# iracigt/ceres-raytracer

Measured on AMD Instinct MI355X. Metric: Mrays/sec (primary+shadow) on dragon.obj 1920x1080; 1/2/4/8-GPU scaling, higher is better.
Workload: dtype f32; 1 GPU; dragon_1080: dragon.obj 1920x1080 primary+shadow, 16 copies of the config view per step; views=config, W=1920, H=1080, row_block=1080, parallelism=one GPU, whole frames, float_framebuffer=True, streams=8

## Files before the change

### ceres-raytracer_amd/csrc/ceres_types.hpp

```cpp
#pragma once
#include <cstddef>
#include <cstdint>
#include <vector>

namespace ceres {

struct Tri48 {
    float p0[3], e1[3], e2[3], n[3];
};
static_assert(sizeof(Tri48) == 48, "Tri48");

struct RefNode {
    float bounds[6];
    uint32_t primitive_count;
    uint32_t first_child_or_primitive;
};
static_assert(sizeof(RefNode) == 32, "RefNode");

struct alignas(16) SiblingPair {
    float lb[6];
    float rb[6];
    uint32_t lcount, lfirst;
    uint32_t rcount, rfirst;
};
// ... 67 lines not shown
    uint32_t error;
    unsigned long long hits;
    unsigned long long pairs;
    unsigned long long tests;
    uint32_t pad[24];
};
static_assert(sizeof(Shard) == 128, "Shard");

constexpr int kMaxFrames = 64;
constexpr int kFramesPerLaunch = 56;
struct FrameCam {
    float eye[3], dir[3], iu[3], iv[3], sun[3];
};

constexpr uint32_t kTileXBits = 13, kTileYBits = 13;
constexpr uint32_t pack_tile(uint32_t f, uint32_t y, uint32_t x) { return (f << (kTileXBits + kTileYBits)) | (y << kTileXBits) | x; }

struct CullRect { uint16_t i0, i1, j0, j1; };

struct KParams {
    FrameCam cam[kFramesPerLaunch];
    CullRect cull_rect[kFramesPerLaunch];
    uint32_t frames;
    uint32_t W, H;
    uint32_t row_block, rank, world, local_rows;
    uint32_t bands;
    uint32_t band_magic;
    uint32_t row_blocks_per_frame;
    uint32_t stack_entries;
    uint32_t root_leaf_count, root_leaf_first;
    float root_box[6];
    uint32_t root_box_ok;
    uint32_t cull;
    uint32_t shadow_stack_entries;
    uint32_t steal_first;
    uint32_t packets;
    uint32_t tiles_x;
    uint32_t lds_entries;
    uint32_t tile_packed;
    const uint32_t* tile_order;
    const SiblingPair* pairs;
    const Node4* nodes4;
    const QNode4* qnodes4;
    const Tri48* tris;
    const uint32_t* orig;
    const float* norms;
    float* pixels;
    uint8_t* rgb8;
    Shard* shards;
    int32_t* rec_prim;
    float* rec_tuv;
    int8_t* rec_shadow;
    unsigned long long* wave_log;
};
static_assert(sizeof(KParams) <= 4096, "KParams must fit the 4 KB kernel-argument limit");

struct DeviceLayout {
    float root_box[6] = {0, 0, 0, 0, 0, 0};
    SiblingPair* pairs = nullptr;
    Node4* nodes4 = nullptr;
    Tri48* tris = nullptr;
    uint32_t* orig = nullptr;
    size_t n_pairs = 0, n_nodes4 = 0;
    uint32_t depth = 0, stack4 = 0, root_leaf_count = 0, root_leaf_first = 0;
};
#ifdef __HIPCC__
int relayout_device(const Tri48* d_tris, uint32_t n_tri, const RefNode* d_nodes, uint32_t n_nodes, const uint32_t* d_prim,
                    hipStream_t stream, DeviceLayout& out);
#endif

int relayout_bvh(const RefNode* nodes, size_t n_nodes, const uint64_t* prim, size_t n_tri, const Tri48* tris,
                 std::vector<SiblingPair>& pairs, std::vector<Tri48>& leaf_tris, std::vector<uint32_t>& orig,
                 uint32_t& depth, uint32_t& root_leaf_count, uint32_t& root_leaf_first);
int build_shadow_bvh4(const std::vector<SiblingPair>& pairs, std::vector<Node4>& out, uint32_t& stack_bound,
                      uint32_t& not_collapsed);
int order_shadow_bvh4(std::vector<Node4>& nodes, uint32_t& first_bound);
int relayout_bvh64(const RefNode64* nodes, size_t n_nodes, const uint64_t* prim, size_t n_tri, const Tri96* tris,
                   std::vector<SiblingPair64>& pairs, std::vector<Tri96>& leaf_tris, std::vector<uint32_t>& orig,
                   uint32_t& depth, uint32_t& root_leaf_count, uint32_t& root_leaf_first);

}
```

### ceres-raytracer_amd/csrc/render_hip.hip

```cpp
#include <hip/hip_runtime.h>

#include <algorithm>
#include <chrono>
#include <cfloat>
#include <cmath>
#include <cstdint>
#include <cstdlib>
#include <cstring>
#include <new>
#include <string>
#include <type_traits>
#include <vector>

#include "ceres_render.h"
#include "ceres_types.hpp"
#include "host_common.hpp"
#include "pow24.hpp"

#pragma clang fp contract(off)

#ifndef CERES_COUNTING
#define CERES_COUNTING 0
#endif
#ifndef CERES_TILES_PER_WAVE
// ... 693 lines not shown
            --sp;
            m = (uint64_t(uint32_t(__builtin_amdgcn_readlane(s_hi, int(sp)))) << 32 |
                 uint32_t(__builtin_amdgcn_readlane(s_lo, int(sp)))) & ~occ;
            if (m) { cur = uint32_t(__builtin_amdgcn_readlane(s_node, int(sp))); break; }
        }
        if (!m) return occ;
    }
}

__device__ __forceinline__ uint8_t quantize(float x) {
    const float a = x * 255;
    const float m = (255.0f < a) ? 255.0f : a;
    const float q = (m < 0.0f) ? 0.0f : m;
    return static_cast<uint8_t>(static_cast<int>(q));
}

__device__ __forceinline__ void store_pixel(const KParams& P, uint32_t f, uint32_t lr, uint32_t i, float c0, float c1,
                                            float c2) {
    const size_t frame_base = size_t(f) * P.local_rows;
    CERES_COUNT_V(kFStoreV, (P.pixels ? 12u : 0u) + (P.rgb8 ? 3u : 0u));
    if (P.pixels) {
        float* q = P.pixels + 3 * ((frame_base + lr) * P.W + i);
        q[0] = c0; q[1] = c1; q[2] = c2;
    }
    if (P.rgb8) {
        uint8_t* q = P.rgb8 + 3 * ((frame_base + (P.local_rows - 1 - lr)) * P.W + i);
        q[0] = quantize(c0); q[1] = quantize(c1); q[2] = quantize(c2);
    }
}

template <bool kBands = false>
__device__ __forceinline__ uint32_t global_row(const KParams& P, uint32_t f, uint32_t lr) {
    if (P.world == 1) return lr;
    if constexpr (kBands) {
        const uint32_t x = P.rank + f, q = __umulhi(x, P.band_magic);
        return (x - q * P.world) * P.row_block + lr;
    }
    return ((lr / P.row_block) * P.world + P.rank) * P.row_block + lr % P.row_block;
}

template <bool kG = false>
__device__ __forceinline__ F3 primary_dir(const KParams& P, uint32_t f, uint32_t i, uint32_t j) {
    const float u = 2 * (float(i) + 0.5f) / float(P.W) - 1.0f;
    const float v = 2 * (float(j) + 0.5f) / float(P.H) - 1.0f;
    const FrameCam& c = P.cam[f];
    F3 a;
    if constexpr (kG)
        a = F3{c.dir[0] + __builtin_fmaf(c.iv[0], v, c.iu[0] * u), c.dir[1] + __builtin_fmaf(c.iv[1], v, c.iu[1] * u),
               c.dir[2] + __builtin_fmaf(c.iv[2], v, c.iu[2] * u)};
    else a = f3(c.iu) * u + f3(c.iv) * v + f3(c.dir);
    return kG ? normalizeG<kG>(a) : normalize(a);
}

__device__ __forceinline__ bool tile_misses_root(const KParams& P, uint32_t f, bool active, uint32_t i, uint32_t j) {
    const CullRect& r = P.cull_rect[f];
    const bool out = i < r.i0 || i > r.i1 || j < r.j0 || j > r.j1;
    return __ballot(active && !out) == 0;
}

template <bool kG>
__device__ __forceinline__ F3 hit_point(const TriV& tr, F3 normal, float hu, float hv) {
    const F3 p1 = tr.p0 - tr.e1, p2 = tr.p0 + tr.e2;
    const float scale = -0.00001;
    const float w = 1 - hu - hv;
    if constexpr (kG) {
        auto c = [&](float p0, float q1, float q2, float n) {
            return __builtin_fmaf(n, scale, __builtin_fmaf(w, q2, __builtin_fmaf(hv, q1, hu * p0)));
        };
        return {c(tr.p0.x, p1.x, p2.x, normal.x), c(tr.p0.y, p1.y, p2.y, normal.y), c(tr.p0.z, p1.z, p2.z, normal.z)};
    } else {
        F3 p = tr.p0 * hu + p1 * hv + p2 * w;
        return p + normal * scale;
    }
}

template <bool kG = false>
__device__ __forceinline__ void shade(F3 sun_line, const float* nrm, F3 view, float u, float v, float c[3]) {
    c[0] = c[1] = c[2] = 0.0f;
    const float amb = 0.2;
    const F3 vneg = view * -1.0f;
    const float w[3] = {u, v, 1 - u - v};
#pragma unroll
    for (int k = 0; k < 3; ++k) {
        const F3 N{nrm[3 * k], nrm[3 * k + 1], nrm[3 * k + 2]};
        const float lam = kG ? fabsf(dotA<true>(sun_line, N)) : fabsf(sun_line.x * N.x + sun_line.y * N.y + sun_line.z * N.z);
        const float spec = 0.8f * pow24f(dotA<kG>(N, normalizeG<kG>(sun_line + vneg)));
        const float base = kG ? __builtin_fmaf(lam, 0.5f, amb) : amb + 0.5f * lam;
        auto clamp01 = [](float x) { return (x < 0.f) ? 0.f : (1.f < x) ? 1.f : x; };
        auto ch = [&](float k) { return kG ? __builtin_fmaf(base, k, spec) : base * k + spec; };
        c[0] += w[k] * clamp01(ch(0.5f));
        c[1] += w[k] * clamp01(ch(0.0f));
        c[2] += w[k] * clamp01(ch(0.8f));
    }
}

__device__ __forceinline__ uint32_t wave_sum(uint32_t x) {
#pragma unroll
    for (int off = 32; off > 0; off >>= 1) x += __shfl_xor(x, off, 64);
    return x;
}

template <bool kStats, bool kRobust, bool kG>
__global__ __launch_bounds__(kBlock) void ceres_primary(const KParams P) {
    extern __shared__ __attribute__((aligned(16))) uint32_t lds[];
    const uint32_t tid = threadIdx.x, lane = tid & 63, wave = tid >> 6;
    uint32_t* stk = lds + tid;
    const uint32_t f = blockIdx.y / P.row_blocks_per_frame;
    const uint32_t by = blockIdx.y - f * P.row_blocks_per_frame;
    const uint32_t lx = lane & 7, ly = lane >> 3;
    const uint32_t i = blockIdx.x * 16 + (wave & 1) * 8 + lx;
    const uint32_t lr = by * 16 + (wave >> 1) * 8 + ly;
    const bool active = i < P.W && lr < P.local_rows;
    const uint32_t px = (f * P.local_rows + lr) * P.W + i;
    bool hit = false;
    Hit h{0, 0.f, 0.f, 0.f};
    uint32_t n_pairs = 0, n_tests = 0;
    bool overflow = false;
    const bool culled = !kStats && P.cull && tile_misses_root(P, f, active, i, global_row(P, f, lr));
    if (culled) {
        if (active) store_pixel(P, f, lr, i, 0.f, 0.f, 0.f);
    } else if (active) {
        const F3 view = primary_dir<kG>(P, f, i, global_row(P, f, lr));
        hit = guarded_trace<kStats, kBlock, uint32_t*, kRobust, -1, kG>(P, f3(P.cam[f].eye), view, stk, h, n_pairs, n_tests,
                                                                      overflow);
        if (P.rec_prim) {
            P.rec_prim[px] = hit ? int32_t(P.orig[h.slot]) : -1;
            P.rec_tuv[3 * size_t(px)] = hit ? h.t : 0.f;
            P.rec_tuv[3 * size_t(px) + 1] = hit ? h.u : 0.f;
            P.rec_tuv[3 * size_t(px) + 2] = hit ? h.v : 0.f;
            P.rec_shadow[px] = -1;
        }
        if (!hit) {
            store_pixel(P, f, lr, i, 0.f, 0.f, 0.f);
        } else {
            CERES_COUNT_V(kFShadeV, 48);
            const F3 normal = normalizeG<kG>(load_tri(P.tris + h.slot).n);
            store_pixel(P, f, lr, i, fabsf(normal.x), fabsf(normal.y), fabsf(normal.z));
        }
    }
    const uint32_t wave_id = (blockIdx.y * gridDim.x + blockIdx.x) * (kBlock / 64) + wave;
    const uint32_t shard = wave_id % kShards;
    const uint32_t nh = __popcll(__ballot(hit));
    if (lane == 0 && nh) atomicAdd(&P.shards[shard].hits, (unsigned long long)nh);
    if (kStats) {
        const uint32_t wp = wave_sum(n_pairs), wt = wave_sum(n_tests);
        if (lane == 0) {
            atomicAdd(&P.shards[shard].pairs, (unsigned long long)wp);
            atomicAdd(&P.shards[shard].tests, (unsigned long long)wt);
        }
    }
    if (overflow) atomicOr(&P.shards[shard].error, 1u);
}

#ifndef CERES_LEAN_WRITES
#define CERES_LEAN_WRITES 0
#endif
#ifndef CERES_FUSED_MINW16
#define CERES_FUSED_MINW16 7
#endif
#ifndef CERES_FUSED_MINW16_TPW4
#define CERES_FUSED_MINW16_TPW4 6
#endif
#ifndef CERES_FUSED_MINW16_SOLO
#define CERES_FUSED_MINW16_SOLO 7
#endif
#ifndef CERES_FUSED_MINW32
#define CERES_FUSED_MINW32 1
#endif
#ifndef CERES_STACK16
#define CERES_STACK16 1
#endif
#ifndef CERES_STACK24
#define CERES_STACK24 1
#endif
// ... 162 lines not shown
    return w;
}

template <typename StkT, bool kRobust, bool kQ, bool kG>
__device__ __forceinline__ bool shadow_packet(const KParams& P, bool hit, const RayWork& w, uint32_t lane, bool& blocked) {
    if constexpr (!kRobust && !kQ && CERES_SHADOW_PACKET && std::is_same<StkT, uint16_t*>::value) {
        const uint64_t act = __ballot(hit);
        if (!act) { blocked = false; return true; }
        const uint32_t oct = (__float_as_uint(w.ix) >> 31) | (__float_as_uint(w.iy) >> 31) << 1 |
                             (__float_as_uint(w.iz) >> 31) << 2;
        const int first = __builtin_ctzll(act);
        const uint32_t oct0 = uint32_t(__builtin_amdgcn_readlane(int(oct), first));
        const bool finite = isfinite(w.ix) && isfinite(w.iy) && isfinite(w.iz) && isfinite(w.sx) && isfinite(w.sy) &&
                            isfinite(w.sz);
        if (!P.packets || P.shadow_stack_entries > 64 || P.root_leaf_count || __ballot(hit && (oct != oct0 || !finite)))
            return false;
        auto bc = [&](float x) { return hit ? x : __int_as_float(__builtin_amdgcn_readlane(__float_as_int(x), first)); };
        const F3 o{bc(w.o.x), bc(w.o.y), bc(w.o.z)}, d{bc(w.d.x), bc(w.d.y), bc(w.d.z)};
        const Slab<false> sl{bc(w.ix), bc(w.iy), bc(w.iz), bc(w.sx), bc(w.sy), bc(w.sz), o};
        uint64_t occ = 0;
        switch (oct0) {
            case 0: occ = packet_any4<0, kG>(P, sl, o, d, act, lane); break;
            case 1: occ = packet_any4<1, kG>(P, sl, o, d, act, lane); break;
            case 2: occ = packet_any4<2, kG>(P, sl, o, d, act, lane); break;
            case 3: occ = packet_any4<3, kG>(P, sl, o, d, act, lane); break;
            case 4: occ = packet_any4<4, kG>(P, sl, o, d, act, lane); break;
            case 5: occ = packet_any4<5, kG>(P, sl, o, d, act, lane); break;
            case 6: occ = packet_any4<6, kG>(P, sl, o, d, act, lane); break;
            default: occ = packet_any4<7, kG>(P, sl, o, d, act, lane); break;
        }
        blocked = (occ >> lane) & 1u;
        return true;
    }
    return false;
}

template <bool kG, bool kBands = false>
__device__ __forceinline__ void shade_pixel(const KParams& P, uint32_t f, uint32_t lr, uint32_t i, uint32_t pix,
                                            bool blocked, F3 sun_line, uint32_t slot, float hu, float hv,
                                            uint32_t& occluded, float c[3]) {
    if (P.rec_shadow) P.rec_shadow[pix] = blocked ? 1 : 0;
    c[0] = c[1] = c[2] = 0.f;
    if (blocked) {
        ++occluded;
    } else {
        const F3 view = primary_dir<kG>(P, f, i, global_row<kBands>(P, f, lr));
        CERES_COUNT_V(kFShadeV, 40);
        shade<kG>(sun_line, P.norms + 9 * size_t(P.orig[slot]), view, hu, hv, c);
    }
}

constexpr int kFusedB = 64;
constexpr size_t kLdsPerCu = 160 * 1024;
__device__ __forceinline__ float fresh_zero() {
    float z;
    asm volatile("v_mov_b32 %0, 0" : "=v"(z));
    return z;
}

template <bool kStats, typename StkT, int kMinW, bool kRobust, bool kSteal, bool kQ, bool kG, int kTPWo = 0, bool kBands = false>
__global__ __launch_bounds__(kFusedB) __attribute__((amdgpu_waves_per_eu(kMinW))) void ceres_fused(const KParams P) {
    constexpr int kB = kFusedB;
    constexpr bool kPacketsCompiled = !kStats && !kSteal && !kRobust && !kQ && CERES_SHADOW_PACKET && std::is_same<StkT, uint16_t*>::value;
    extern __shared__ __attribute__((aligned(16))) uint32_t lds[];
    __shared__ StealLdsT<kB> L;
    const uint32_t lane = threadIdx.x, tid = lane;
    constexpr uint32_t kTPWp = (kStats || kSteal) ? 1 : kTPWo ? uint32_t(kTPWo) : uint32_t(CERES_TILES_PER_WAVE);
    constexpr bool kPair = CERES_PAIR_STORES && !kStats && !kSteal && kTPWp >= 2 && std::is_same<StkT, uint16_t*>::value;
    __shared__ typename std::conditional<kPair, PairStash, NoStash>::type S;
    auto tile_pixel = [&](uint32_t t, uint32_t& f_, uint32_t& lr_, uint32_t& i_) {
        uint32_t by_, bx_;
        if (P.tile_packed) {
            bx_ = t & ((1u << kTileXBits) - 1u);
            by_ = (t >> kTileXBits) & ((1u << kTileYBits) - 1u);
            f_ = t >> (kTileXBits + kTileYBits);
        } else {
            const uint32_t per_frame_ = P.tiles_x * P.row_blocks_per_frame;
            f_ = t / per_frame_;
            const uint32_t rem = t - f_ * per_frame_;
            by_ = rem / P.tiles_x; bx_ = rem - by_ * P.tiles_x;
        }
        const uint32_t lx = (lane & 1) | ((lane >> 1) & 2) | ((lane >> 2) & 4), ly = ((lane >> 1) & 1) | ((lane >> 2) & 2) | ((lane >> 3) & 4);
        i_ = bx_ * 8u + lx;
        lr_ = by_ * 8u + ly;
        return i_ < P.W && lr_ < P.local_rows && (!kBands || global_row<true>(P, f_, lr_) < P.H);
    };
    auto emit = [&](uint32_t q, bool last, uint32_t t_prev, bool act, uint32_t f_, uint32_t lr_, uint32_t i_, float c0, float c1,
                    float c2) {
        if constexpr (kPair) {
            if (!(q & 1u) && !last) {
                S.c[0][lane] = c0; S.c[1][lane] = c1; S.c[2][lane] = c2;
                return;
            }
            if (q & 1u) {
                uint32_t pf, plr, pi;
                if (tile_pixel(t_prev, pf, plr, pi)) store_pixel(P, pf, plr, pi, S.c[0][lane], S.c[1][lane], S.c[2][lane]);
            }
        }
        if (act) store_pixel(P, f_, lr_, i_, c0, c1, c2);
    };
    StkT stk;
    if constexpr (std::is_same<StkT, Stk24>::value)
        stk = Stk24{reinterpret_cast<uint16_t*>(lds) + tid,
                    reinterpret_cast<uint8_t*>(lds) + size_t(P.lds_entries) * kB * 2 + tid};
    else
        stk = reinterpret_cast<StkT>(lds) + tid;
    constexpr uint32_t kTile = 8;
    constexpr uint32_t kTPW = (kStats || kSteal) ? 1 : kTPWo ? uint32_t(kTPWo) : uint32_t(CERES_TILES_PER_WAVE);
    const uint32_t per_frame = P.tiles_x * P.row_blocks_per_frame;
    const uint32_t n_tiles = per_frame * P.frames;
    uint32_t n_shadow = 0, occluded = 0, n_pairs = 0, n_tests = 0;
    bool overflow = false;
    static_assert(kTPW == 1 || kTPW == 2 || kTPW == 4 || kTPW == 8, "CERES_TILES_PER_WAVE must be 1, 2, 4 or 8");
    uint4 tiles4 = make_uint4(0, 0, 0, 0), tiles4b = make_uint4(0, 0, 0, 0);
    if constexpr (kTPW == 8) {
        tiles4 = sload_u4(P.tile_order + 8 * size_t(blockIdx.x), 0);
        tiles4b = sload_u4(P.tile_order + 8 * size_t(blockIdx.x), 1);
    } else if constexpr (kTPW == 4) {
        tiles4 = sload_u4(P.tile_order + 4 * size_t(blockIdx.x), 0);
    } else if constexpr (kTPW == 2) {
        tiles4.x = sload_u32(P.tile_order + 2 * size_t(blockIdx.x));
        tiles4.y = sload_u32(P.tile_order + 2 * size_t(blockIdx.x) + 1);
    } else {
        tiles4.x = sload_u32(P.tile_order + blockIdx.x);
    }
    CERES_COUNT_S(kFOrderS, 4 * kTPW);
    for (uint32_t q = 0; q < kTPW; ++q) {
    const uint32_t slot_q = blockIdx.x * kTPW + q;
    if (kTPW > 1 && slot_q >= n_tiles) break;
    const uint4 tq = q < 4 ? tiles4 : tiles4b;
    const uint32_t qq = q & 3;
    const uint32_t t = kTPW == 1 ? tiles4.x : qq == 0 ? tq.x : qq == 1 ? tq.y : qq == 2 ? tq.z : tq.w;
    const uint32_t qp = (q - 1) & 3;
    const uint4 tp = q - 1 < 4 ? tiles4 : tiles4b;
    const uint32_t t_prev = qp == 0 ? tp.x : qp == 1 ? tp.y : qp == 2 ? tp.z : tp.w;
    uint32_t f, lr, i;
    bool active = tile_pixel(t, f, lr, i);
    uint32_t px = (f * P.local_rows + lr) * P.W + i;
    auto redecode = [&]() {
        if constexpr (CERES_LEAN_WRITES) {
            uint32_t tr = t;
            asm volatile("" : "+s"(tr));
            active = tile_pixel(tr, f, lr, i);
            px = (f * P.local_rows + lr) * P.W + i;
        }
    };
    bool hit = false;
    Hit h{0, 0.f, 0.f, 0.f};
    RayWork w{};
    uint64_t t_start = 0;
    if (kStats && P.wave_log) t_start = __builtin_amdgcn_s_memrealtime();
    const bool last_q = q + 1 == kTPW || (kTPW > 1 && slot_q + 1 >= n_tiles);
    if (!kStats && P.cull && tile_misses_root(P, f, active, i, global_row<kBands>(P, f, lr))) {
        const float z = CERES_LEAN_WRITES ? fresh_zero() : 0.f;
        emit(q, last_q, t_prev, active, f, lr, i, z, z, z);
        continue;
    }
    if (active) {
        const F3 view = primary_dir<kG>(P, f, i, global_row<kBands>(P, f, lr));
        constexpr int kOctMode = (!kSteal || (CERES_OCTANT_SLAB & 4)) ? -1 : -2;
        hit = guarded_trace<kStats, kB, StkT, kRobust, kOctMode, kG>(P, f3(P.cam[f].eye), view, stk, h, n_pairs,
                                                                   n_tests, overflow);
        if (P.rec_prim) {
            redecode();
            P.rec_prim[px] = hit ? int32_t(P.orig[h.slot]) : -1;
            P.rec_tuv[3 * size_t(px)] = hit ? h.t : 0.f;
            P.rec_tuv[3 * size_t(px) + 1] = hit ? h.u : 0.f;
            P.rec_tuv[3 * size_t(px) + 2] = hit ? h.v : 0.f;
            P.rec_shadow[px] = -1;
        }
        if (hit) {
            CERES_COUNT_V(kFShadeV, 48);
            const TriV tr = load_tri(P.tris + h.slot);
            const F3 normal = normalizeG<kG>(tr.n);
            w = make_shadow_ray<kRobust, kG>(hit_point<kG>(tr, normal, h.u, h.v), f3(P.cam[f].sun));
        }
    }
    const uint32_t n_shadow_t = __popcll(__ballot(hit));
    n_shadow += n_shadow_t;
    uint64_t t_primary = 0;
    uint32_t prim_pairs = n_pairs, shadow_iters = 0;
    if (kStats && P.wave_log) t_primary = __builtin_amdgcn_s_memrealtime();
    bool pk_blocked = false;
    const bool pk = !kStats && !kSteal && shadow_packet<StkT, kRobust, kQ, kG>(P, hit, w, lane, pk_blocked);
    if (pk)
        L.blocked[tid] = pk_blocked ? 1u : 0u;
    else if constexpr (kSteal)
        steal_traverse<kStats, kB, StkT, kRobust, kQ, kG>(P, hit, w, stk, L, tid, lane, n_pairs, n_tests, overflow, &shadow_iters);
    else
        L.blocked[tid] = hit && trace_any4<kStats, kB, StkT, kRobust, kQ, kPacketsCompiled ? -2 : -1, kG>(
                                    P, w.o, w.d, stk, n_pairs, n_tests, overflow) ? 1u : 0u;
    redecode();
    float col[3] = {0.f, 0.f, 0.f};
    if (hit) shade_pixel<kG, kBands>(P, f, lr, i, px, L.blocked[tid] != 0, w.d, h.slot, h.u, h.v, occluded, col);
    emit(q, last_q, t_prev, active, f, lr, i, col[0], col[1], col[2]);
    if (kStats && P.wave_log) {
        const uint64_t t_end = __builtin_amdgcn_s_memrealtime();
        uint32_t mx = prim_pairs;
        for (int off = 32; off > 0; off >>= 1) mx = max(mx, uint32_t(__shfl_xor(int(mx), off, 64)));
        const uint32_t sp = wave_sum(prim_pairs), ss = wave_sum(n_pairs - prim_pairs);
        if (lane == 0) {
            unsigned long long* wl = P.wave_log + 8 * size_t(blockIdx.x);
            wl[0] = t_start; wl[1] = t_primary; wl[2] = t_end; wl[3] = mx; wl[4] = shadow_iters;
            wl[5] = n_shadow_t; wl[6] = sp; wl[7] = ss;
        }
    }
    }
    const uint32_t wo = wave_sum(occluded);
// ... 496 lines not shown
int build_qnodes4(ceres_scene* s) {
    if (!s->n_nodes4 || !s->d_nodes4) return CERES_OK;
    std::vector<Node4> n4(s->n_nodes4);
    HIP_TRY(hipMemcpy(n4.data(), s->d_nodes4, n4.size() * sizeof(Node4), hipMemcpyDeviceToHost));
    std::vector<QNode4> q;
    if (int rc = quantize_nodes4(n4, q)) return rc;
    HIP_TRY(hipMalloc(&s->d_qnodes4, q.size() * sizeof(QNode4)));
    HIP_TRY(hipMemcpy(s->d_qnodes4, q.data(), q.size() * sizeof(QNode4), hipMemcpyHostToDevice));
    return CERES_OK;
}

void set_root_box(ceres_scene* s, const float root[6], const SiblingPair& p0) {
    for (int k = 0; k < 6; ++k) s->root_box[k] = root[k];
    auto inside = [&](const float* c) {
        return c[0] >= root[0] && c[1] <= root[1] && c[2] >= root[2] && c[3] <= root[3] && c[4] >= root[4] && c[5] <= root[5];
    };
    s->root_box_ok = (!s->root_leaf_count && inside(p0.lb) && inside(p0.rb)) ? 1u : 0u;
}

static CullRect cull_rect(const FrameCam& c, const float root[6], uint32_t W, uint32_t H) {
    const CullRect keep{0u, 0xffffu, 0u, 0xffffu};
    if (W > 0xffffu || H > 0xffffu) return keep;
    double e[3], iu[3], iv[3], d[3];
    for (int k = 0; k < 3; ++k) { e[k] = c.eye[k]; iu[k] = c.iu[k]; iv[k] = c.iv[k]; d[k] = c.dir[k]; }
    double sc = 0;
    for (int k = 0; k < 3; ++k) sc = std::max(sc, std::fabs(e[k]));
    for (int k = 0; k < 6; ++k) sc = std::max(sc, std::fabs(double(root[k])));
    const double pad = 1e-4 * sc;
    auto cr = [](const double* a, const double* b, double* o) {
        o[0] = a[1] * b[2] - a[2] * b[1]; o[1] = a[2] * b[0] - a[0] * b[2]; o[2] = a[0] * b[1] - a[1] * b[0]; };
    double c0[3], c1[3], c2[3];
    cr(iv, d, c0); cr(d, iu, c1); cr(iu, iv, c2);
    const double det = iu[0] * c0[0] + iu[1] * c0[1] + iu[2] * c0[2];
    double u0 = HUGE_VAL, u1 = -HUGE_VAL, v0 = HUGE_VAL, v1 = -HUGE_VAL;
    for (int k = 0; k < 8; ++k) {
        const double X[3] = {(k & 1) ? root[1] + pad : root[0] - pad, (k & 2) ? root[3] + pad : root[2] - pad,
                             (k & 4) ? root[5] + pad : root[4] - pad};
        const double r[3] = {X[0] - e[0], X[1] - e[1], X[2] - e[2]};
        const double pw = r[0] * c0[0] + r[1] * c0[1] + r[2] * c0[2], qw = r[0] * c1[0] + r[1] * c1[1] + r[2] * c1[2];
        const double ww = r[0] * c2[0] + r[1] * c2[1] + r[2] * c2[2];
        if (!(ww / det > 0.01 * std::sqrt(r[0] * r[0] + r[1] * r[1] + r[2] * r[2]))) return keep;
        u0 = std::min(u0, pw / ww); u1 = std::max(u1, pw / ww); v0 = std::min(v0, qw / ww); v1 = std::max(v1, qw / ww);
    }
    const double m = 2e-3 * (1 + std::max(std::max(std::fabs(u0), std::fabs(u1)), std::max(std::fabs(v0), std::fabs(v1))));
    auto lo = [](double x, uint32_t n) { return x <= 0 ? 0u : x >= n ? n : uint32_t(std::floor(x)); };
    const double a0 = (u0 - m + 1) * W / 2 - 0.5 - 1, a1 = (u1 + m + 1) * W / 2 - 0.5 + 1;
    const double b0 = (v0 - m + 1) * H / 2 - 0.5 - 1, b1 = (v1 + m + 1) * H / 2 - 0.5 + 1;
    if (!(a0 == a0 && a1 == a1 && b0 == b0 && b1 == b1)) return keep;
    if (a1 < 0 || b1 < 0) return CullRect{1u, 0u, 1u, 0u};
    return CullRect{uint16_t(lo(a0, W)), uint16_t(std::min<double>(std::ceil(a1), 0xffff)),
                    uint16_t(lo(b0, H)), uint16_t(std::min<double>(std::ceil(b1), 0xffff))};
}

static int stack_width(size_t n_pairs, size_t n_nodes4) {
    const size_t nmax = std::max(n_pairs, n_nodes4);
    return CERES_STACK16 && nmax < (1u << 16) ? 2 : CERES_STACK24 && nmax < (1u << 24) ? 3 : 4;
}
static uint32_t batch_tiles_per_wave(size_t frame_pixels, int stw, bool qbvh) {
    if (!CERES_TPW_BY_SIZE || stw != 2 || qbvh) return CERES_TILES_PER_WAVE;
    return frame_pixels >= (size_t(1) << 20) && frame_pixels < (size_t(1) << 22) ? 2u : uint32_t(CERES_TILES_PER_WAVE);
}

static size_t fused_lds_bytes(uint32_t entries, int stw) {
    return size_t(entries) * dev::kFusedB * stw + sizeof(dev::StealLdsT<dev::kFusedB>);
}
static bool lds_limits_waves(uint32_t entries, int stw) { return fused_lds_bytes(entries, stw) > dev::kLdsPerCu / 28; }

static int check_fused_lds(const ceres_scene* s, const KParams& P, int stw, size_t dyn_bytes) {
    const size_t need = size_t(P.lds_entries) * dev::kFusedB * size_t(stw);
    const size_t total = dyn_bytes + sizeof(dev::StealLdsT<dev::kFusedB>);
    if (stw != 2 && stw != 3 && stw != 4)
        return set_error(CERES_EINVAL, "render: bad LDS stack entry width %d", stw);
    if (P.lds_entries < P.stack_entries + 1 || P.lds_entries < P.shadow_stack_entries || dyn_bytes < need)
        return set_error(CERES_EINVAL, "render: LDS stack of %u slots (%zu B) cannot hold the BVH2 stack (%u + 1) and the BVH4 "
                         "stack (%u)", P.lds_entries, dyn_bytes, P.stack_entries, P.shadow_stack_entries);
    if (total > s->max_lds_per_block)
        return set_error(CERES_EINVAL, "render: fused kernel needs %zu B of LDS per workgroup (%zu available)", total,
                         s->max_lds_per_block);
    return CERES_OK;
}

int launch_chunk(ceres_scene* s, uint32_t frames, const float* basis12, const float* sun, int mode, size_t W, size_t H,
                 const ceres_tiling* tiling, float* d_pixels, uint8_t* d_rgb8, uint64_t* d_counters, hipStream_t stream,
                 int32_t* d_rec_prim, float* d_rec_tuv, int8_t* d_rec_shadow, bool first, bool last,
                 uint64_t batch_primary) {
    if (!s || !basis12 || !sun) return set_error(CERES_EINVAL, "render: null argument");
    if (s->f64) return set_error(CERES_EINVAL, "scene is double precision: use ceres_render_f64");
    if (frames == 0 || frames > uint32_t(kFramesPerLaunch))
        return set_error(CERES_EINVAL, "render: %u frames per launch (1..%d)", frames, kFramesPerLaunch);
    const bool robust = (mode & CERES_MODE_ROBUST) != 0;
    const bool qbvh = (mode & CERES_MODE_QBVH4) != 0;
    const bool gfma = (mode & CERES_MODE_FMA) != 0;
    mode &= ~(CERES_MODE_ROBUST | CERES_MODE_QBVH4 | CERES_MODE_FMA);
    if (mode != CERES_MODE_FULL && mode != CERES_MODE_PRIMARY) return set_error(CERES_EINVAL, "render: bad mode %d", mode);
    if (W == 0 || H == 0 || W > 65535u * 16u || H > 0xffffffu) return set_error(CERES_EINVAL, "render: bad size %zux%zu", W, H);
    ceres_tiling t{uint32_t(H), 0, 1};
    if (tiling) t = *tiling;
    if (t.world == 0 || t.rank >= t.world || t.row_block == 0) return set_error(CERES_EINVAL, "render: bad tiling");
    if (t.world == 1) t.bands = 0;
    if (t.bands && (t.bands != 1 || t.world > 65535u || size_t(t.row_block) * t.world < H))
        return set_error(CERES_EINVAL, "render: bands of %u rows x %u ranks do not cover %zu rows", t.row_block, t.world, H);
    const size_t rows = local_rows_of(H, t);
    if (size_t(frames) * W * rows > 0xffffffffull) return set_error(CERES_EINVAL, "render: more than 2^32 pixels per batch");
    const uint32_t bx = uint32_t((W + 15) / 16), by = uint32_t((rows + 15) / 16);
    if (size_t(by) * frames > 65535u) return set_error(CERES_EINVAL, "render: frames x row blocks exceeds the grid limit");
    if ((d_rec_prim != nullptr) != (d_rec_tuv != nullptr) || (d_rec_prim != nullptr) != (d_rec_shadow != nullptr))
        return set_error(CERES_EINVAL, "render: hit records need all three arrays");
    if (qbvh && (robust || (s->flags & CERES_SCENE_STATS)))
        return set_error(CERES_EUNSUPPORTED, "render: CERES_MODE_QBVH4 takes neither CERES_MODE_ROBUST nor a stats scene");
    if (t.bands && (mode != CERES_MODE_FULL || robust || qbvh || (s->flags & CERES_SCENE_STATS) || d_rec_prim))
        return set_error(CERES_EUNSUPPORTED, "render: ceres_tiling.bands takes the full mode of a non-stats scene "
                                             "(not ROBUST, QBVH4, PRIMARY or hit records)");
    HIP_TRY(hipSetDevice(s->device));
    if (qbvh && mode == CERES_MODE_FULL && !s->d_qnodes4)
        if (int rc = build_qnodes4(s)) return rc;

    KParams P{};
    for (uint32_t f = 0; f < frames; ++f) {
        FrameCam& c = P.cam[f];
        std::memcpy(c.eye, basis12 + 12 * f, 12); std::memcpy(c.dir, basis12 + 12 * f + 3, 12);
        std::memcpy(c.iu, basis12 + 12 * f + 6, 12); std::memcpy(c.iv, basis12 + 12 * f + 9, 12);
        std::memcpy(c.sun, sun + 3 * f, 12);
    }
    P.frames = frames;
    P.W = uint32_t(W); P.H = uint32_t(H);
    P.row_block = t.row_block; P.rank = t.rank; P.world = t.world; P.local_rows = uint32_t(rows);
    P.bands = t.bands;
    P.band_magic = t.bands ? uint32_t(((uint64_t(1) << 32) + t.world - 1) / t.world) : 0u;
    P.row_blocks_per_frame = by;
    P.stack_entries = s->stack_entries;
    P.shadow_stack_entries = s->shadow_stack_entries;
    P.packets = (s->n_pairs * sizeof(SiblingPair) + s->n_nodes4 * sizeof(Node4) + s->n_tri * sizeof(Tri48)) <
                kDramSceneBytes ? 1u : 0u;
    P.root_leaf_count = s->root_leaf_count; P.root_leaf_first = s->root_leaf_first;
    for (int k = 0; k < 6; ++k) P.root_box[k] = s->root_box[k];
    P.root_box_ok = CERES_ROOT_TEST ? s->root_box_ok : 0u;
    P.cull = (CERES_CULL && P.root_box_ok && !(s->flags & CERES_SCENE_STATS) && !d_rec_prim) ? 1u : 0u;
    if (P.cull)
        for (uint32_t f = 0; f < frames; ++f) P.cull_rect[f] = cull_rect(P.cam[f], P.root_box, P.W, P.H);
    P.pairs = s->d_pairs; P.nodes4 = s->d_nodes4; P.tris = s->d_tris; P.orig = s->d_orig; P.norms = s->d_norms;
    P.qnodes4 = s->d_qnodes4;
    P.pixels = d_pixels; P.rgb8 = d_rgb8; P.shards = s->d_shards;
    P.rec_prim = d_rec_prim; P.rec_tuv = d_rec_tuv; P.rec_shadow = d_rec_shadow;

    const bool stats = (s->flags & CERES_SCENE_STATS) != 0;
    const bool full = mode == CERES_MODE_FULL;
    hipEvent_t e0 = nullptr, e1 = nullptr;
    if (s->timing && rows) {
        while (s->ev_pool.size() < 2) { hipEvent_t e; HIP_TRY(hipEventCreate(&e)); s->ev_pool.push_back(e); }
        e0 = s->ev_pool.back(); s->ev_pool.pop_back();
        e1 = s->ev_pool.back(); s->ev_pool.pop_back();
        s->ev_used.push_back(e0); s->ev_used.push_back(e1);
    }
    constexpr uint32_t ftile = 8;
    const uint32_t fbx = uint32_t((W + ftile - 1) / ftile), fby = uint32_t((rows + ftile - 1) / ftile);
    const uint32_t* tile_order = nullptr;
    const bool packed = frames <= (1u << (32 - kTileXBits - kTileYBits)) &&
                        fbx <= (1u << kTileXBits) && fby <= (1u << kTileYBits);
    const uint32_t tpw = (!stats && (frames > 1 || t.bands)) ? batch_tiles_per_wave(size_t(W) * rows, stack_width(s->n_pairs, s->n_nodes4), qbvh)
                                                : 1u;
    if (full && rows)
        if (int rc = ensure_tile_order(s, W, H, t, rows, frames, fbx, fby, ftile, stream, &tile_order, packed, tpw)) return rc;
    const bool need_clean = d_counters || !full;
    if (first && need_clean && s->shards_dirty) HIP_TRY(hipMemsetAsync(s->d_shards, 0, sizeof(Shard) * kShards, stream));
    s->shards_dirty = true;
    if (rows) {
        if (e0) HIP_TRY(hipEventRecord(e0, stream));
        if (full) {
            const int stw = stack_width(s->n_pairs, s->n_nodes4);
            const bool st16 = stw == 2;
            const bool steal = frames == 1 && !t.bands;
            P.steal_first = steal && !stats && ((s->flags & CERES_SCENE_FIRST_ORDER) ||
                                                lds_limits_waves(std::max(s->stack_entries + 1, s->shadow_stack_entries), stw))
                                ? 1u : 0u;
            P.shadow_stack_entries = (!steal || P.steal_first) ? s->shadow_stack_first : s->shadow_stack_entries;
            P.lds_entries = uint32_t(std::max(s->stack_entries + 1, P.shadow_stack_entries));
            const size_t flds = size_t(P.lds_entries) * dev::kFusedB * stw;
            if (int rc = check_fused_lds(s, P, stw, flds)) return rc;
            if (!stats)
                if (const char* g = std::getenv("CERES_DEBUG_GUARD_SLOT")) {
                    const long k = std::strtol(g, nullptr, 10);
                    if (k > 0 && uint32_t(k) < P.stack_entries) P.stack_entries = uint32_t(k);
                }
            P.tile_order = tile_order;
            P.tile_packed = packed ? 1u : 0u;
            P.tiles_x = fbx;
            P.row_blocks_per_frame = fby;
            const uint32_t n_tiles = fbx * fby * frames;
            const dim3 fgrid((n_tiles + tpw - 1) / tpw), fblock(dev::kFusedB);
            if (stats) {
                const size_t waves = size_t(fbx) * fby * frames;
                if (s->wave_log_waves < waves) {
                    dfree(s->d_wave_log);
                    HIP_TRY(hipMalloc(&s->d_wave_log, waves * 64));
                    s->wave_log_waves = waves;
                }
                HIP_TRY(hipMemsetAsync(s->d_wave_log, 0, waves * 64, stream));
                P.wave_log = s->d_wave_log;
                s->last_grid_waves = waves;
            }
            constexpr int w32 = CERES_FUSED_MINW32;
            auto fused = [&](auto rt, auto st, auto gt) {
                constexpr bool R = decltype(rt)::value, T = decltype(st)::value, G = decltype(gt)::value;
                constexpr int w16 = T ? CERES_FUSED_MINW16_SOLO : CERES_FUSED_MINW16;
                if constexpr (!R) {
                    if (qbvh) {
                        if (st16) hipLaunchKernelGGL((dev::ceres_fused<false, uint16_t*, w16, false, T, true, G>), fgrid, fblock, flds, stream, P);
                        else if (stw == 3) hipLaunchKernelGGL((dev::ceres_fused<false, dev::Stk24, w32, false, T, true, G>), fgrid, fblock, flds, stream, P);
                        else hipLaunchKernelGGL((dev::ceres_fused<false, uint32_t*, w32, false, T, true, G>), fgrid, fblock, flds, stream, P);
                        return;
                    }
                }
                if (stats && st16) hipLaunchKernelGGL((dev::ceres_fused<true, uint16_t*, 1, R, T, false, G>), fgrid, fblock, flds, stream, P);
                else if (stats && stw == 3) hipLaunchKernelGGL((dev::ceres_fused<true, dev::Stk24, w32, R, T, false, G>), fgrid, fblock, flds, stream, P);
                else if (stats) hipLaunchKernelGGL((dev::ceres_fused<true, uint32_t*, w32, R, T, false, G>), fgrid, fblock, flds, stream, P);
                else if (st16) {
                    if constexpr (!T) {
                        if (tpw == 2) { hipLaunchKernelGGL((dev::ceres_fused<false, uint16_t*, w16, R, T, false, G, 2>), fgrid, fblock, flds, stream, P); return; }
                    }
                    constexpr int w16b = T ? CERES_FUSED_MINW16_SOLO : CERES_FUSED_MINW16_TPW4;
                    hipLaunchKernelGGL((dev::ceres_fused<false, uint16_t*, w16b, R, T, false, G>), fgrid, fblock, flds, stream, P);
                }
                else if (stw == 3) hipLaunchKernelGGL((dev::ceres_fused<false, dev::Stk24, w32, R, T, false, G>), fgrid, fblock, flds, stream, P);
                else hipLaunchKernelGGL((dev::ceres_fused<false, uint32_t*, w32, R, T, false, G>), fgrid, fblock, flds, stream, P);
            };
            auto fused_g = [&](auto rt, auto st) {
                if (gfma) fused(rt, st, std::true_type{});
                else fused(rt, st, std::false_type{});
            };
            auto fused_s = [&](auto rt) {
                if (steal) fused_g(rt, std::true_type{});
                else fused_g(rt, std::false_type{});
            };
            auto fused_bands = [&](auto gt) {
                constexpr bool G = decltype(gt)::value;
                if (st16) {
                    if (tpw == 2) hipLaunchKernelGGL((dev::ceres_fused<false, uint16_t*, CERES_FUSED_MINW16, false, false, false, G, 2, true>), fgrid, fblock, flds, stream, P);
                    else hipLaunchKernelGGL((dev::ceres_fused<false, uint16_t*, CERES_FUSED_MINW16_TPW4, false, false, false, G, 0, true>), fgrid, fblock, flds, stream, P);
                } else if (stw == 3) hipLaunchKernelGGL((dev::ceres_fused<false, dev::Stk24, w32, false, false, false, G, 0, true>), fgrid, fblock, flds, stream, P);
                else hipLaunchKernelGGL((dev::ceres_fused<false, uint32_t*, w32, false, false, false, G, 0, true>), fgrid, fblock, flds, stream, P);
            };
            if (t.bands) {
                if (gfma) fused_bands(std::true_type{});
                else fused_bands(std::false_type{});
            } else if (robust) fused_s(std::true_type{});
            else fused_s(std::false_type{});
        } else {
            const size_t lds = size_t(s->stack_entries + 1) * dev::kBlock * 4;
            if (lds > s->max_lds_per_block)
                return set_error(CERES_EINVAL, "render: primary-only traversal stack needs %zu B of LDS per workgroup (%zu available)",
                                 lds, s->max_lds_per_block);
            const dim3 grid(bx, by * frames), block(dev::kBlock);
            auto primary = [&](auto rt, auto gt) {
                constexpr bool R = decltype(rt)::value, G = decltype(gt)::value;
                if (stats) hipLaunchKernelGGL((dev::ceres_primary<true, R, G>), grid, block, lds, stream, P);
                else hipLaunchKernelGGL((dev::ceres_primary<false, R, G>), grid, block, lds, stream, P);
            };
            auto primary_g = [&](auto rt) {
                if (gfma) primary(rt, std::true_type{});
                else primary(rt, std::false_type{});
            };
            if (robust) primary_g(std::true_type{});
            else primary_g(std::false_type{});
        }
        HIP_TRY(hipGetLastError());
        if (e1) HIP_TRY(hipEventRecord(e1, stream));
    }
    if (d_counters && last) {
        hipLaunchKernelGGL(dev::ceres_finalize, dim3(1), dim3(64), 0, stream, s->d_shards,
                           batch_primary, d_counters);
        HIP_TRY(hipGetLastError());
        s->shards_dirty = false;
    }
    return CERES_OK;
}

int launch(ceres_scene* s, uint32_t frames, const float* basis12, const float* sun, int mode, size_t W, size_t H,
           const ceres_tiling* tiling, float* d_pixels, uint8_t* d_rgb8, uint64_t* d_counters, hipStream_t stream,
           int32_t* d_rec_prim = nullptr, float* d_rec_tuv = nullptr, int8_t* d_rec_shadow = nullptr) {
    if (frames == 0 || frames > uint32_t(kMaxFrames))
        return set_error(CERES_EINVAL, "render: %u frames per batch (1..%d)", frames, kMaxFrames);
    if (!basis12 || !sun) return set_error(CERES_EINVAL, "render: null argument");
    ceres_tiling t{uint32_t(H), 0, 1};
    if (tiling) t = *tiling;
    if (t.world == 0 || t.rank >= t.world || t.row_block == 0) return set_error(CERES_EINVAL, "render: bad tiling");
    uint64_t primary = uint64_t(frames) * W * local_rows_of(H, t);
    if (t.bands && t.world > 1) {
        primary = 0;
        for (uint32_t f = 0; f < frames; ++f) {
            const size_t b = (t.rank + f) % t.world, top = b * size_t(t.row_block);
            primary += uint64_t(W) * (top < H ? std::min<size_t>(t.row_block, H - top) : 0);
        }
    }
    if (frames <= uint32_t(kFramesPerLaunch))
        return launch_chunk(s, frames, basis12, sun, mode, W, H, tiling, d_pixels, d_rgb8, d_counters, stream, d_rec_prim,
                            d_rec_tuv, d_rec_shadow, true, true, primary);
    const size_t fp = W * local_rows_of(H, t);
    const uint32_t n_launch = (frames + kFramesPerLaunch - 1) / kFramesPerLaunch;
    for (uint32_t c = 0, f0 = 0; c < n_launch; ++c) {
        const uint32_t n = frames / n_launch + (c < frames % n_launch ? 1u : 0u);
        const size_t o = size_t(f0) * fp;
        ceres_tiling tc = t;
        if (t.bands) tc.rank = (t.rank + f0) % t.world;
        if (int rc = launch_chunk(s, n, basis12 + 12 * size_t(f0), sun + 3 * size_t(f0), mode, W, H, &tc,
                                  d_pixels ? d_pixels + 3 * o : nullptr, d_rgb8 ? d_rgb8 + 3 * o : nullptr, d_counters,
// ... 788 lines not shown
```

Measured before the change: 47700 Mrays/s.

## Offload culled-tile zero fills to dedicated fill waves with coalesced vector stores

Tiles whose 8x8 footprint misses the root bounding box no longer write per-pixel zeros inside the trace loop. Extra workgroups are appended to the grid, optionally interleaved among tile groups through a magic-number stride. Each zeroes whole culled row runs with aligned 16-byte stores. The host disables culling when no tile would be culled, which adds a host-side pre-scan. Risks include extra grid blocks, duplicated indexing logic between host and device, and correctness subtleties in the pair-stash flush handling.

```diff
diff --git a/ceres-raytracer_amd/csrc/ceres_types.hpp b/ceres-raytracer_amd/csrc/ceres_types.hpp
--- a/ceres-raytracer_amd/csrc/ceres_types.hpp
+++ b/ceres-raytracer_amd/csrc/ceres_types.hpp
@@ -143,6 +143,7 @@
     float* rec_tuv;
     int8_t* rec_shadow;
     unsigned long long* wave_log;
+    uint32_t fill_stride, fill_magic;
 };
 static_assert(sizeof(KParams) <= 4096, "KParams must fit the 4 KB kernel-argument limit");
 
diff --git a/ceres-raytracer_amd/csrc/render_hip.hip b/ceres-raytracer_amd/csrc/render_hip.hip
--- a/ceres-raytracer_amd/csrc/render_hip.hip
+++ b/ceres-raytracer_amd/csrc/render_hip.hip
@@ -769,10 +769,87 @@
     return kG ? normalizeG<kG>(a) : normalize(a);
 }
 
-__device__ __forceinline__ bool tile_misses_root(const KParams& P, uint32_t f, bool active, uint32_t i, uint32_t j) {
+
+__host__ __device__ inline bool cull_cols_hit(const CullRect& r, uint32_t W, uint32_t bx) {
+    const uint32_t a = 8u * bx, b = a + 7u < W - 1u ? a + 7u : W - 1u;
+    const uint32_t lo = a > r.i0 ? a : uint32_t(r.i0), hi = b < r.i1 ? b : uint32_t(r.i1);
+    return lo <= hi;
+}
+template <bool kBands = false>
+__device__ __forceinline__ bool row_exists(const KParams& P, uint32_t f, uint32_t lr) {
+    return lr < P.local_rows && (!kBands || global_row<true>(P, f, lr) < P.H);
+}
+template <bool kBands = false>
+__device__ __forceinline__ bool tile_rows_hit(const KParams& P, uint32_t f, uint32_t lr) {
     const CullRect& r = P.cull_rect[f];
-    const bool out = i < r.i0 || i > r.i1 || j < r.j0 || j > r.j1;
-    return __ballot(active && !out) == 0;
+    const uint32_t j = global_row<kBands>(P, f, lr);
+    return __ballot(row_exists<kBands>(P, f, lr) && j >= r.j0 && j <= r.j1) != 0;
+}
+__device__ __forceinline__ bool tile_misses_root(const KParams& P, uint32_t f, uint32_t bx, bool rows_hit) {
+    return !(rows_hit && cull_cols_hit(P.cull_rect[f], P.W, bx));
+}
+
+template <typename T>
+__device__ __forceinline__ void zero_run(T* p, size_t n, uint32_t lane) {
+    static_assert(16 % sizeof(T) == 0, "zero_run");
+    if (!n) return;
+    CERES_COUNT_S(kFStoreV, uint32_t(n * sizeof(T)));
+    const uint32_t mis = uint32_t(reinterpret_cast<uintptr_t>(p)) & 15u;
+    size_t head = mis ? (16u - mis) / sizeof(T) : 0u;
+    if (head > n) head = n;
+    if (lane < head) p[lane] = T(0);
+    p += head; n -= head;
+    const size_t nv = n * sizeof(T) / 16;
+    uint4* v = reinterpret_cast<uint4*>(p);
+    for (size_t k = lane; k < nv; k += 64) v[k] = make_uint4(0u, 0u, 0u, 0u);
+    const size_t done = nv * (16 / sizeof(T));
+    if (lane < n - done) p[done + lane] = T(0);
+}
+
+#ifndef CERES_FILL_SPREAD
+#define CERES_FILL_SPREAD 1
+#endif
+
+template <bool kBands = false>
+__device__ __forceinline__ void fill_culled_rows(const KParams& P, uint32_t task, uint32_t lane) {
+    const uint32_t tile_rows = (P.local_rows + 7u) / 8u, tiles_x = (P.W + 7u) / 8u;
+    const uint32_t f = task / tile_rows, by = task - f * tile_rows;
+    if (f >= P.frames) return;
+    const uint32_t lr = by * 8u + (lane & 7u);
+    const uint32_t n = __popcll(__ballot(lane < 8u && row_exists<kBands>(P, f, lr)));
+    if (!n) return;
+    const bool rows_hit = tile_rows_hit<kBands>(P, f, lr);
+    uint32_t bx0 = 0, bx1 = 0;
+    bool any = false;
+    for (uint32_t base = 0; base < tiles_x; base += 64u) {
+        const uint64_t m = __ballot(base + lane < tiles_x && !tile_misses_root(P, f, base + lane, rows_hit));
+        if (m) {
+            if (!any) bx0 = base + uint32_t(__builtin_ctzll(m));
+            bx1 = base + 63u - uint32_t(__builtin_clzll(m));
+            any = true;
+        }
+    }
+    const size_t W = P.W, frame_base = size_t(f) * P.local_rows;
+    if (!any) {
+        const size_t lo = by * 8u, hi = lo + n - 1;
+        if (P.pixels) zero_run(P.pixels + 3 * ((frame_base + lo) * W), 3 * n * W, lane);
+        if (P.rgb8) zero_run(P.rgb8 + 3 * ((frame_base + (P.local_rows - 1 - hi)) * W), 3 * n * W, lane);
+        return;
+    }
+    const size_t a = size_t(bx0) * 8u, b = size_t(bx1) * 8u + 8u < W ? size_t(bx1) * 8u + 8u : W;
+    for (uint32_t k = 0; k < n; ++k) {
+        const size_t row = by * 8u + k;
+        if (P.pixels) {
+            float* q = P.pixels + 3 * ((frame_base + row) * W);
+            zero_run(q, 3 * a, lane);
+            zero_run(q + 3 * b, 3 * (W - b), lane);
+        }
+        if (P.rgb8) {
+            uint8_t* q = P.rgb8 + 3 * ((frame_base + (P.local_rows - 1 - row)) * W);
+            zero_run(q, 3 * a, lane);
+            zero_run(q + 3 * b, 3 * (W - b), lane);
+        }
+    }
 }
 
 template <bool kG>
@@ -821,6 +898,11 @@
 __global__ __launch_bounds__(kBlock) void ceres_primary(const KParams P) {
     extern __shared__ __attribute__((aligned(16))) uint32_t lds[];
     const uint32_t tid = threadIdx.x, lane = tid & 63, wave = tid >> 6;
+    if (!kStats && blockIdx.y >= P.frames * P.row_blocks_per_frame) {
+        const uint32_t g = (blockIdx.y - P.frames * P.row_blocks_per_frame) * gridDim.x + blockIdx.x;
+        fill_culled_rows(P, g * (kBlock / 64) + wave, lane);
+        return;
+    }
     uint32_t* stk = lds + tid;
     const uint32_t f = blockIdx.y / P.row_blocks_per_frame;
     const uint32_t by = blockIdx.y - f * P.row_blocks_per_frame;
@@ -833,10 +915,8 @@
     Hit h{0, 0.f, 0.f, 0.f};
     uint32_t n_pairs = 0, n_tests = 0;
     bool overflow = false;
-    const bool culled = !kStats && P.cull && tile_misses_root(P, f, active, i, global_row(P, f, lr));
-    if (culled) {
-        if (active) store_pixel(P, f, lr, i, 0.f, 0.f, 0.f);
-    } else if (active) {
+    const bool culled = !kStats && P.cull && tile_misses_root(P, f, i >> 3, tile_rows_hit(P, f, lr));
+    if (!culled && active) {
         const F3 view = primary_dir<kG>(P, f, i, global_row(P, f, lr));
         hit = guarded_trace<kStats, kBlock, uint32_t*, kRobust, -1, kG>(P, f3(P.cam[f].eye), view, stk, h, n_pairs, n_tests,
                                                                       overflow);
@@ -1105,12 +1185,6 @@
 
 constexpr int kFusedB = 64;
 constexpr size_t kLdsPerCu = 160 * 1024;
-__device__ __forceinline__ float fresh_zero() {
-    float z;
-    asm volatile("v_mov_b32 %0, 0" : "=v"(z));
-    return z;
-}
-
 template <bool kStats, typename StkT, int kMinW, bool kRobust, bool kSteal, bool kQ, bool kG, int kTPWo = 0, bool kBands = false>
 __global__ __launch_bounds__(kFusedB) __attribute__((amdgpu_waves_per_eu(kMinW))) void ceres_fused(const KParams P) {
     constexpr int kB = kFusedB;
@@ -1138,17 +1212,23 @@
         lr_ = by_ * 8u + ly;
         return i_ < P.W && lr_ < P.local_rows && (!kBands || global_row<true>(P, f_, lr_) < P.H);
     };
+    bool stashed = false;
+    auto flush = [&](uint32_t t_prev) {
+        if constexpr (kPair) {
+            uint32_t pf, plr, pi;
+            if (tile_pixel(t_prev, pf, plr, pi)) store_pixel(P, pf, plr, pi, S.c[0][lane], S.c[1][lane], S.c[2][lane]);
+        }
+        stashed = false;
+    };
     auto emit = [&](uint32_t q, bool last, uint32_t t_prev, bool act, uint32_t f_, uint32_t lr_, uint32_t i_, float c0, float c1,
                     float c2) {
         if constexpr (kPair) {
             if (!(q & 1u) && !last) {
                 S.c[0][lane] = c0; S.c[1][lane] = c1; S.c[2][lane] = c2;
+                stashed = true;
                 return;
             }
-            if (q & 1u) {
-                uint32_t pf, plr, pi;
-                if (tile_pixel(t_prev, pf, plr, pi)) store_pixel(P, pf, plr, pi, S.c[0][lane], S.c[1][lane], S.c[2][lane]);
-            }
+            if (stashed) flush(t_prev);
         }
         if (act) store_pixel(P, f_, lr_, i_, c0, c1, c2);
     };
@@ -1162,25 +1242,41 @@
     constexpr uint32_t kTPW = (kStats || kSteal) ? 1 : kTPWo ? uint32_t(kTPWo) : uint32_t(CERES_TILES_PER_WAVE);
     const uint32_t per_frame = P.tiles_x * P.row_blocks_per_frame;
     const uint32_t n_tiles = per_frame * P.frames;
+    uint32_t group = blockIdx.x;
+    if constexpr (!kStats) {
+        const uint32_t tile_groups = (n_tiles + kTPW - 1) / kTPW;
+        if (P.fill_stride) {
+            const uint32_t oct = blockIdx.x >> 3, x = blockIdx.x & 7u, nfo = (gridDim.x >> 3) - (tile_groups + 7u) / 8u;
+            const uint32_t q = __umulhi(oct, P.fill_magic), r = oct - q * P.fill_stride;
+            if (r == P.fill_stride - 1 && q < nfo) {
+                fill_culled_rows<kBands>(P, q * 8u + x, lane);
+                return;
+            }
+            group = (oct - (q < nfo ? q : nfo)) * 8u + x;
+            if (group >= tile_groups) return;
+        } else if (blockIdx.x >= tile_groups) {
+            fill_culled_rows<kBands>(P, blockIdx.x - tile_groups, lane);
+            return;
+        }
+    }
     uint32_t n_shadow = 0, occluded = 0, n_pairs = 0, n_tests = 0;
     bool overflow = false;
     static_assert(kTPW == 1 || kTPW == 2 || kTPW == 4 || kTPW == 8, "CERES_TILES_PER_WAVE must be 1, 2, 4 or 8");
     uint4 tiles4 = make_uint4(0, 0, 0, 0), tiles4b = make_uint4(0, 0, 0, 0);
     if constexpr (kTPW == 8) {
-        tiles4 = sload_u4(P.tile_order + 8 * size_t(blockIdx.x), 0);
-        tiles4b = sload_u4(P.tile_order + 8 * size_t(blockIdx.x), 1);
+        tiles4 = sload_u4(P.tile_order + 8 * size_t(group), 0);
+        tiles4b = sload_u4(P.tile_order + 8 * size_t(group), 1);
     } else if constexpr (kTPW == 4) {
-        tiles4 = sload_u4(P.tile_order + 4 * size_t(blockIdx.x), 0);
+        tiles4 = sload_u4(P.tile_order + 4 * size_t(group), 0);
     } else if constexpr (kTPW == 2) {
-        tiles4.x = sload_u32(P.tile_order + 2 * size_t(blockIdx.x));
-        tiles4.y = sload_u32(P.tile_order + 2 * size_t(blockIdx.x) + 1);
+        tiles4.x = sload_u32(P.tile_order + 2 * size_t(group));
+        tiles4.y = sload_u32(P.tile_order + 2 * size_t(group) + 1);
     } else {
-        tiles4.x = sload_u32(P.tile_order + blockIdx.x);
+        tiles4.x = sload_u32(P.tile_order + group);
     }
     CERES_COUNT_S(kFOrderS, 4 * kTPW);
-    for (uint32_t q = 0; q < kTPW; ++q) {
-    const uint32_t slot_q = blockIdx.x * kTPW + q;
-    if (kTPW > 1 && slot_q >= n_tiles) break;
+    const uint32_t n_here = kTPW == 1 || n_tiles - group * kTPW >= kTPW ? kTPW : n_tiles - group * kTPW;
+    for (uint32_t q = 0; q < n_here; ++q) {
     const uint4 tq = q < 4 ? tiles4 : tiles4b;
     const uint32_t qq = q & 3;
     const uint32_t t = kTPW == 1 ? tiles4.x : qq == 0 ? tq.x : qq == 1 ? tq.y : qq == 2 ? tq.z : tq.w;
@@ -1203,10 +1299,9 @@
     RayWork w{};
     uint64_t t_start = 0;
     if (kStats && P.wave_log) t_start = __builtin_amdgcn_s_memrealtime();
-    const bool last_q = q + 1 == kTPW || (kTPW > 1 && slot_q + 1 >= n_tiles);
-    if (!kStats && P.cull && tile_misses_root(P, f, active, i, global_row<kBands>(P, f, lr))) {
-        const float z = CERES_LEAN_WRITES ? fresh_zero() : 0.f;
-        emit(q, last_q, t_prev, active, f, lr, i, z, z, z);
+    const bool last_q = q + 1 == n_here;
+    if (!kStats && P.cull && tile_misses_root(P, f, i >> 3, tile_rows_hit<kBands>(P, f, lr))) {
+        if (stashed) flush(t_prev);
         continue;
     }
     if (active) {
@@ -1809,6 +1904,27 @@
                     uint16_t(lo(b0, H)), uint16_t(std::min<double>(std::ceil(b1), 0xffff))};
 }
 
+static bool launch_culls_a_tile(const KParams& P) {
+    const uint32_t tiles_x = (P.W + 7u) / 8u;
+    for (uint32_t f = 0; f < P.frames; ++f) {
+        const CullRect& r = P.cull_rect[f];
+        const bool all_cols = dev::cull_cols_hit(r, P.W, 0) && dev::cull_cols_hit(r, P.W, tiles_x - 1);
+        for (uint32_t lr0 = 0; lr0 < P.local_rows; lr0 += 8) {
+            bool exists = false, hit = false;
+            for (uint32_t lr = lr0; lr < lr0 + 8 && lr < P.local_rows; ++lr) {
+                const uint32_t j = P.world == 1 ? lr
+                                   : P.bands    ? ((P.rank + f) % P.world) * P.row_block + lr
+                                                : ((lr / P.row_block) * P.world + P.rank) * P.row_block + lr % P.row_block;
+                if (P.bands && P.world > 1 && j >= P.H) continue;
+                exists = true;
+                hit = hit || (j >= r.j0 && j <= r.j1);
+            }
+            if (exists && !(hit && all_cols)) return true;
+        }
+    }
+    return false;
+}
+
 static int stack_width(size_t n_pairs, size_t n_nodes4) {
     const size_t nmax = std::max(n_pairs, n_nodes4);
     return CERES_STACK16 && nmax < (1u << 16) ? 2 : CERES_STACK24 && nmax < (1u << 24) ? 3 : 4;
@@ -1892,9 +2008,13 @@
     P.root_leaf_count = s->root_leaf_count; P.root_leaf_first = s->root_leaf_first;
     for (int k = 0; k < 6; ++k) P.root_box[k] = s->root_box[k];
     P.root_box_ok = CERES_ROOT_TEST ? s->root_box_ok : 0u;
-    P.cull = (CERES_CULL && P.root_box_ok && !(s->flags & CERES_SCENE_STATS) && !d_rec_prim) ? 1u : 0u;
-    if (P.cull)
+    P.cull = (CERES_CULL && P.root_box_ok && !(s->flags & CERES_SCENE_STATS) && !d_rec_prim && W <= 0xffffu && H <= 0xffffu) ? 1u : 0u;
+    uint32_t fill_tasks = 0;
+    if (P.cull) {
         for (uint32_t f = 0; f < frames; ++f) P.cull_rect[f] = cull_rect(P.cam[f], P.root_box, P.W, P.H);
+        if (rows && launch_culls_a_tile(P)) fill_tasks = frames * uint32_t((rows + 7) / 8);
+        else P.cull = 0u;
+    }
     P.pairs = s->d_pairs; P.nodes4 = s->d_nodes4; P.tris = s->d_tris; P.orig = s->d_orig; P.norms = s->d_norms;
     P.qnodes4 = s->d_qnodes4;
     P.pixels = d_pixels; P.rgb8 = d_rgb8; P.shards = s->d_shards;
@@ -1944,7 +2064,16 @@
             P.tiles_x = fbx;
             P.row_blocks_per_frame = fby;
             const uint32_t n_tiles = fbx * fby * frames;
-            const dim3 fgrid((n_tiles + tpw - 1) / tpw), fblock(dev::kFusedB);
+            const uint32_t tile_groups = (n_tiles + tpw - 1) / tpw;
+            dim3 fgrid(tile_groups + fill_tasks), fblock(dev::kFusedB);
+            if (CERES_FILL_SPREAD > (steal ? 1 : 0) && fill_tasks) {
+                const uint64_t nto = (tile_groups + 7) / 8, nfo = (fill_tasks + 7) / 8, stride = (nto + nfo) / nfo;
+                if (stride >= 2 && (nto + nfo) * stride < (uint64_t(1) << 32)) {
+                    fgrid.x = uint32_t((nto + nfo) * 8);
+                    P.fill_stride = uint32_t(stride);
+                    P.fill_magic = uint32_t(((uint64_t(1) << 32) + stride - 1) / stride);
+                }
+            }
             if (stats) {
                 const size_t waves = size_t(fbx) * fby * frames;
                 if (s->wave_log_waves < waves) {
@@ -2007,7 +2136,9 @@
             if (lds > s->max_lds_per_block)
                 return set_error(CERES_EINVAL, "render: primary-only traversal stack needs %zu B of LDS per workgroup (%zu available)",
                                  lds, s->max_lds_per_block);
-            const dim3 grid(bx, by * frames), block(dev::kBlock);
+            uint32_t fill_y = (((fill_tasks + dev::kBlock / 64 - 1) / (dev::kBlock / 64)) + bx - 1) / bx;
+            if (size_t(by) * frames + fill_y > 65535u) { P.cull = 0u; fill_y = 0; }
+            const dim3 grid(bx, by * frames + fill_y), block(dev::kBlock);
             auto primary = [&](auto rt, auto gt) {
                 constexpr bool R = decltype(rt)::value, G = decltype(gt)::value;
                 if (stats) hipLaunchKernelGGL((dev::ceres_primary<true, R, G>), grid, block, lds, stream, P);
```

Result: faster. 49800 Mrays/s (median of 6 runs) (+4.4%).
